# migmolper/NL-PartSol

Measured on AMD Instinct MI355X. Metric: particle-steps/sec (P2G+stress+G2P), higher is better.
Workload: dtype f64; 1 GPU; 3-D elastic cube impact, 1000000 particles/GPU (50x50x50 cells x 8 over 1 rank(s)), LME gamma=3, Neo-Hookean E=1e7 nu=0.3, explicit predictor-corrector step, 1xMI355X per rank; z-slabs for N>1 (weak scaling); particles_total=1000000, grid_nodes=226981, halo=none, halo_impl=none, library_default_resort_interval=50

## Files before the change

### nl-partsol_amd/csrc/nlps_gpu.hip

```cpp
#include <hip/hip_runtime.h>
#include <unistd.h>
#include <thread>
#include <hipcub/hipcub.hpp>

#include <dlfcn.h>
#include <rccl/rccl.h>

#include <algorithm>
#include <cmath>
#include <cstdio>
#include <cstdlib>
#include <cstring>
#include <numeric>
#include <map>
#include <string>
#include <type_traits>
#include <vector>

#include "../../include/nlps_gpu.h"
#include "nlps_device.hpp"
#include "nlps_tables.hpp"
#include "nlps_host_mem.hpp"

#define LAUNCH_ND_BLK(kern2, kern3, grid, block, ...)                                              \
// ... 226 lines not shown
      N.fixed[A * ND + a] = 0;
    }
  }
}

template <int ND>
__device__ __forceinline__ void dilate_node(int A, const GridD& g, const NView& N) {
  const int i0 = A % g.n[0], j0 = (A / g.n[0]) % g.n[1], k0 = A / (g.n[0] * g.n[1]);
  unsigned any = 0u;
#pragma unroll
  for (int dk = (ND == 3 ? -1 : 0); dk <= (ND == 3 ? 1 : 0); dk++)
#pragma unroll
    for (int dj = -1; dj <= 1; dj++)
#pragma unroll
      for (int di = -1; di <= 1; di++) {
        const int i = i0 + di, j = j0 + dj, k = k0 + dk;
        const bool ok = i >= 0 && i < g.n[0] && j >= 0 && j < g.n[1] && (ND == 2 || (k >= 0 && k < g.n[2]));
        if (ok) any |= N.seed[i + g.n[0] * (j + g.n[1] * k)];
      }
  N.active[A] = any ? 1 : 0;
}

template <int ND>
__device__ __forceinline__ int closest_node_update(const GridD& g, const uint8_t* __restrict__ rank1, const double* x, int I0) {
  int ijk[3] = {I0 % g.n[0], (I0 / g.n[0]) % g.n[1], I0 / (g.n[0] * g.n[1])};
  const uint8_t* rk = rank1 + 27 * class3_of<ND>(g, ijk);
  int sgn[3] = {0, 0, 0};
#pragma unroll
  for (int a = 0; a < ND; a++) {
    const double d = x[a] - (g.o[a] + g.h * (double)ijk[a]);
    if (fabs(d) > 0.49 * g.h) sgn[a] = d > 0.0 ? 1 : -1;
  }
  double best = 0.0;
  int bestrank = 256, bi = ijk[0], bj = ijk[1], bk = ijk[2];
#pragma unroll
  for (int q = 0; q < (1 << ND); q++) {
    const int di = (q & 1) ? sgn[0] : 0, dj = (q & 2) ? sgn[1] : 0, dk = (ND == 3 && (q & 4)) ? sgn[2] : 0;
    const bool dup = ((q & 1) && sgn[0] == 0) || ((q & 2) && sgn[1] == 0) || (ND == 3 && (q & 4) && sgn[2] == 0);
    const int i = ijk[0] + di, j = ijk[1] + dj, k = ijk[2] + dk;
    const bool ok = !dup && i >= 0 && i < g.n[0] && j >= 0 && j < g.n[1] && (ND == 2 || (k >= 0 && k < g.n[2]));
    if (ok) {
      double Dc = 0.0, t;
      t = x[0] - (g.o[0] + g.h * (double)i);
      Dc += t * t;
      t = x[1] - (g.o[1] + g.h * (double)j);
      Dc += t * t;
      if (ND == 3) {
        t = x[ND - 1] - (g.o[2] + g.h * (double)k);
        Dc += t * t;
      }
      const double d = sqrt(Dc);
      const int rank = rk[(di + 1) + 3 * (dj + 1) + 9 * (dk + 1)];
      if (bestrank == 256 || d < best || (d == best && rank < bestrank)) {
        best = d;
        bestrank = rank;
        bi = i;
        bj = j;
        bk = k;
      }
    }
  }
  return bi + g.n[0] * (bj + g.n[1] * bk);
}

template <int ND>
__global__ __launch_bounds__(BLK) void k_search(PView P, GridD g, NView N, const uint8_t* __restrict__ rank1, TileCnt tc,
                                                int update) {
  const int p = blockIdx.x * BLK + threadIdx.x;
  const bool valid = p < P.np;
  int I0 = 0;
  if (valid) {
    I0 = P.I0[p];
    if (update) {
      double x[ND], aux = 0.0;
#pragma unroll
      for (int a = 0; a < ND; a++) {
        x[a] = PF(P, F_X + a, p);
        aux += dsqr(PF(P, F_DIS + a, p));
      }
      if (sqrt(aux) > 0.0) {
        I0 = closest_node_update<ND>(g, rank1, x, I0);
        P.I0[p] = I0;
      }
      P.I0n[p] = I0;
    } else {
      const int In = P.I0n[p];
      if (In != I0) P.I0[p] = In;
      I0 = In;
    }
  }
  bin_particle<ND>(P, g, tc, p, I0, valid);
  if (valid && (!tc.count || P.tile[p] >= 0)) N.seed[I0] = 1;
}

template <int ND>
__global__ __launch_bounds__(BLK) void k_search_ahead(PView P, GridD g, NView N, const uint8_t* __restrict__ rank1, TileCnt tc) {
  const int p = blockIdx.x * BLK + threadIdx.x;
  int I0n = 0;
  bool binned = false;
  if (p < P.np) {
    I0n = P.I0[p];
    binned = P.tile[p] >= 0;
    if (binned && (P.mlo[p] | P.mhi[p]) != 0ull) {
      double xn[ND], dn2 = 0.0;
#pragma unroll
      for (int a = 0; a < ND; a++) {
        const double dd = PF(P, F_DDIS + a, p);
        xn[a] = PF(P, F_X + a, p) + dd;
        const double dn = PF(P, F_DIS + a, p) + dd;
        dn2 += dsqr(dn);
      }
      if (sqrt(dn2) > 0.0) I0n = closest_node_update<ND>(g, rank1, xn, I0n);
    }
    P.I0n[p] = I0n;
  }
  bin_particle<ND>(P, g, tc, binned ? p : P.np, I0n, binned);
  if (binned && P.tile[p] >= 0) N.seed[I0n] = 1;
}

__global__ void k_commit_I0(int np, const int* __restrict__ I0n, int* __restrict__ I0) {
  const int p = blockIdx.x * blockDim.x + threadIdx.x;
  if (p < np) I0[p] = I0n[p];
}

template <int ND>
__global__ __launch_bounds__(BLK) void k_init_I0(PView P, GridD g, NView N, TileCnt tc) {
  const int p = blockIdx.x * BLK + threadIdx.x;
  bool valid = p < P.np;
  int bestnode = 0;
  if (valid) {
    double x[ND];
    int c[3] = {0, 0, 0};
    bool found = true;
#pragma unroll
    for (int a = 0; a < ND; a++) {
      x[a] = PF(P, F_X + a, p);
      int nc = g.n[a] - 1;
      int ci = (int)floor((x[a] - g.o[a]) / g.h);
      ci = ci < 0 ? 0 : (ci > nc - 1 ? nc - 1 : ci);
      while (ci > 0 && x[a] <= g.o[a] + g.h * (double)ci) ci--;
// ... 1109 lines not shown
  bool rolled = false;
  bool level_b_fields = false;

  DevBuf<double> gridA;
  DevBuf<double> gridB;
  DevBuf<double> maskedA;

  std::vector<BcDev> bcs;
  DevBuf<unsigned> bcmask_d;

  DevBuf<int> perm_d;
  bool perm_dirty;
  int resort_every, steps_since_sort;
  DevBuf<unsigned long long> skey_d, skey2_d;
  DevBuf<int> sval_d, sval2_d;
  DevBuf<char> cub_tmp;
  size_t cub_tmp_bytes = 0;
  DevBuf<double> gather_tmp;
  DevBuf<double> Pd_alt;

  int nt[3], ntiles;
  DevBuf<int> tile_count_d;
  DevBuf<int> tile_count2_d;
  DevBuf<int> tile_start_d;
  DevBuf<int2> work1_d;
  DevBuf<int> node_cnt_d, nrank_d, tabo_d;
  DevBuf<int> tile_cursor_d;
  bool ranks_deferred = false;
  DevBuf<unsigned long long> tabm_d;
  DevBuf<int> home_d, foreign_d;
  Pinned<int> foreign_h;
  Pinned<int> status_h;
  bool rehome = true;
  double adaptive_resort = 0.8, debt = 0.0;
  int adaptive_min_steps = 4;
  DevBuf<int> nwork_d;
  DevBuf<int> dmg_first_d, dmg_last_d;
  DevBuf<int> dmg_first0_d, dmg_last0_d, dmg_sorted0_d;
  bool beps_snapshot = false;
  bool explicit_damage = false;
  int xl_n = 0, xl_nloads = 0;
  double xl_thickness = 1.0;
  DevBuf<int> xl_ids_d, xl_load_d, xl_inv_d;
  DevBuf<double> xl_a0_d, xl_T_d;
  bool xl_inv_valid = false, xl_lane_map = false;
  hipEvent_t xl_ev[2] = {};
// ... 399 lines not shown
  h->prm.tol_wrapper = prm->tol_wrapper_lme;
  h->prm.max_iter_lme = prm->max_iter_lme;
  h->prm.tol_radial = prm->tol_radial_returning;
  h->prm.max_iter_radial = prm->max_iter_radial_returning;
  h->P.erosion = prm->driver_eigenerosion != 0 || prm->driver_eigensoftening != 0;
  h->P.softening = prm->driver_eigensoftening != 0 && prm->driver_eigenerosion == 0;
#if NLPS_DEV
  if (const char* e = getenv("NLPS_LAZY_NODAL")) h->lazy_nodal = atoi(e);
#endif
  {
    int dev = 0, ncu = 0;
    if (hipGetDevice(&dev) == hipSuccess && hipDeviceGetAttribute(&ncu, hipDeviceAttributeMultiprocessorCount, dev) == hipSuccess && ncu > 0)
      h->ncu = ncu;
  }

  h->tab = nlps_host::build_tables(g.nd);
  HIPCHK(h->rank1_d.reserve(27 * 27));
  HIPCHK(hipMemcpy(h->rank1_d, h->tab.rank1, 27 * 27, hipMemcpyHostToDevice));

  size_t nn = (size_t)g.nnodes;
  int ND = g.nd;
  if (dev_alloc(h, h->N_active, nn, &h->N.active)) return 1;
  if (dev_alloc(h, h->N_seed, nn, &h->N.seed)) return 1;
  if (dev_alloc(h, h->N_nm, nn * (1 + ND), &h->N.nm)) return 1;
  if (dev_alloc(h, h->N_dU, nn * ND, &h->N.dU)) return 1;
  if (dev_alloc(h, h->N_force, nn * ND, &h->N.force)) return 1;
  if (dev_alloc(h, h->N_accel, nn * ND, &h->N.accel)) return 1;
  if (dev_alloc(h, h->N_reaction, nn * ND, &h->N.reaction)) return 1;
  if (dev_alloc(h, h->N_fixed, nn * ND, &h->N.fixed)) return 1;
  if (dev_alloc(h, h->h_avg_d, nn)) return 1;
  if (dev_alloc(h, h->n2m_d, nn)) return 1;
  if (dev_alloc(h, h->d2m_d, nn * ND)) return 1;
  if (dev_alloc(h, h->fixedm_d, nn * ND)) return 1;
  if (dev_alloc(h, h->bsum_d, nn * ND / 1024 + 2)) return 1;
  if (dev_alloc(h, h->total_d, 4)) return 1;
  if (dev_alloc(h, h->gstatus_d, 4)) return 1;
  if (dev_alloc(h, h->gridA, nn * 2 * ND)) return 1;
  if (dev_alloc(h, h->gridB, nn * 4 * ND)) return 1;
  {
    std::vector<double> hv;
    if (grid->h_avg) hv.assign(grid->h_avg, grid->h_avg + nn);
    else host_h_avg(*grid, h->tab, hv);
    HIPCHK(hipMemcpy(h->h_avg_d, hv.data(), nn * sizeof(double), hipMemcpyHostToDevice));
    h->N.h_avg = h->h_avg_d;
    HIPCHK(h->beta_t2_d.reserve(nn));
    hipLaunchKernelGGL(k_node_tables, dim3(nblk((int)nn)), dim3(BLK), 0, 0, (int)nn, (const double*)h->h_avg_d,
// ... 68 lines not shown
        used += m != 0;
        mixed += (m & (m - 1)) != 0;
      }
      h->k3_per_law = used > 0 && 4 * mixed <= used;
      if (h->law_present & ((1 << NLPS_KLAW_FRICTIONAL) | (1 << NLPS_KLAW_FLUID))) h->k3_per_law = 1;
    }
    std::stable_sort(h->perm.begin(), h->perm.end(), [&](int a, int b) { return key[a] < key[b]; });
    h->slab_lo = std::max(0, lo - 3);
    h->slab_hi = std::min(g.n[slab_axis] - 1, hi + 3);
  }
  if (dev_alloc(h, h->Pd, (size_t)NFD * h->P.npad, &h->P.d)) return 1;
  if (dev_alloc(h, h->P_I0, h->P.npad, &h->P.I0)) return 1;
  if (dev_alloc(h, h->P_I0n, h->P.npad, &h->P.I0n)) return 1;
  if (dev_alloc(h, h->P_mat, h->P.npad, &h->P.mat)) return 1;
  if (dev_alloc(h, h->P_nn, h->P.npad, &h->P.nn)) return 1;
  if (dev_alloc(h, h->P_status, h->P.npad, &h->P.status)) return 1;
  if (dev_alloc(h, h->P_mlo, h->P.npad, &h->P.mlo)) return 1;
  if (dev_alloc(h, h->P_mhi, h->P.npad, &h->P.mhi)) return 1;
  if (dev_alloc(h, h->P_tile, h->P.npad, &h->P.tile)) return 1;
  if (dev_alloc(h, h->P_rank, h->P.npad, &h->P.rank)) return 1;
  if (dev_alloc(h, h->order_d, h->P.npad)) return 1;
  if (dev_alloc(h, h->tile_count_d, (size_t)h->ntiles + 1)) return 1;
  if (dev_alloc(h, h->tile_count2_d, (size_t)h->ntiles + 1)) return 1;
  if (dev_alloc(h, h->tile_start_d, (size_t)h->ntiles + 1)) return 1;
  if (dev_alloc(h, h->work1_d, (size_t)h->ntiles)) return 1;
  if (dev_alloc(h, h->nwork_d, 6)) return 1;
#if NLPS_DEV
  if (const char* e = getenv("NLPS_ADAPTIVE_RESORT")) h->adaptive_resort = atof(e);
#endif
  if (dev_alloc(h, h->node_cnt_d, (size_t)h->g.nnodes)) return 1;
  if (dev_alloc(h, h->nrank_d, h->P.npad)) return 1;
  if (dev_alloc(h, h->tile_cursor_d, (size_t)h->ntiles + 1)) return 1;
  {
    const size_t nnw = h->g.nd == 3 ? TileTabCfg<3>::NNW : TileTabCfg<2>::NNW;
    if (dev_alloc(h, h->tabo_d, (size_t)h->ntiles * TileTab::LMAX * nnw)) return 1;
    if (dev_alloc(h, h->tabm_d, (size_t)h->ntiles * TileTab::LMAX * nnw)) return 1;
  }
  if (dev_alloc(h, h->home_d, h->P.npad)) return 1;
  if (dev_alloc(h, h->foreign_d, 64 * 32)) return 1;
  HIPCHK(h->foreign_h.alloc());
  *h->foreign_h.host() = 0;
  HIPCHK(h->status_h.alloc());
  *h->status_h.host() = 0;
#if NLPS_PHASE_TIMING
  if (dev_alloc(h, h->phase_d, 16 * 1024)) return 1;
#endif
  {
    std::vector<double> tmp(h->P.npad);
    int T = h->T;
    double idrow[9] = {0};
    idrow[0] = 1.0;
    idrow[ND + 1] = 1.0;
    idrow[T - 1] = 1.0;
// ... 1315 lines not shown
      td.slab_slot = -1;
      for_each_law_present(h->law_present, [&](int l, bool) {
        td.slab_slot++;
        launch_k3_law<MODE, true, 64>(h, td, l, a.dV);
      });
      return;
    }
  }
  if (per_law) {
    for_each_law_present(h->law_present, [&](int l, bool last) {
      if (a.signal && last) arm_signal(h, td, 1);
      launch_k3_law<MODE, true, K3_BLK>(h, td, l, a.dV);
    });
  } else if (law < 0) {
    if constexpr (K3Forms<MODE>::dispatch) {
      with_nd(h->nd, [&](auto D) { k3_go(h, k3_tile<CT(D), -1, MODE>, K3_BLK, td, no_rates); });
    }
  } else if (one_material_3d(h)) {
    with_law_in<1, 3>(law, [&](auto L) { k3_go(h, k3_tile<3, CT(L), MODE, false, K3_BLK, true>, K3_BLK, td, no_rates); });
  } else {
    launch_k3_law<MODE, false, K3_BLK>(h, td, law, a.dV);
  }
}
static void launch_k3_lazy(nlps_gpu* h, TileD td, bool signal, const LazyNodal& ln) {
  if (signal) arm_signal(h, td, 1);
  if (one_material_3d(h)) {
    with_law_in<1, 3>(h->uniform_law, [&](auto L) { k3_go(h, k3_tile_lazy<3, CT(L), true>, K3_BLK, td, ln); });
  } else {
    with_nd(h->nd, [&](auto D) {
      with_law(h->uniform_law, [&](auto L) { k3_go(h, k3_tile_lazy<CT(D), CT(L)>, K3_BLK, td, ln); });
    });
  }
}

template <int NF2, int NF3>
static void det_gather(nlps_gpu* h, int part, int slab_count, double* out) {
  const NodeRanges r = node_ranges(h, part);
  TileD tg = tile_view(h, 0);
  tg.slab_n = slab_count;
  if (r.an + r.bn > 0)
    LAUNCH_ND((k_slab_gather<2, NF2>), (k_slab_gather<3, NF3>), nblk(r.an + r.bn), r.a0, r.an, r.b0, r.bn, h->g, tg, out);
}
template <int NF2, int NF3, class F>
static int scatter_tiles(nlps_gpu* h, const char* who, int slab_count, double* out, F&& launch) {
  if (!det_implicit(h)) {
    launch(ic<BLK>{}, tile_view(h));
    return 0;
  }
  if (det_prepare(h, who)) return 1;
  launch(ic<64>{}, tile_view(h));
  det_gather<NF2, NF3>(h, 0, slab_count, out);
  return 0;
}
// ... 8 lines not shown
  }
  with_nd(h->nd, [&](auto D) {
    with_bool(p2g, [&](auto P2G) {
      hipLaunchKernelGGL((k2_tile<CT(D), CT(P2G)>), dim3(h->ntw), dim3(BLK), 0, h->stream, h->P, h->g, h->N, td,
                         h->prm, dt, gamma_nm, h->gstatus_d);
    });
  });
}

static int ensure_list_twins(nlps_gpu* h) {
  if (h->order_2_d) return 0;
  const size_t nn = (size_t)h->g.nnodes, ND = (size_t)h->nd;
  if (dev_alloc(h, h->work1_2_d, (size_t)h->ntiles)) return 1;
  if (dev_alloc(h, h->nwork2_d, 6)) return 1;
  if (dev_alloc(h, h->tile_start2_d, (size_t)h->ntiles + 1)) return 1;
  if (dev_alloc(h, h->order2_2_d, h->P.npad)) return 1;
  if (dev_alloc(h, h->N_active2, nn)) return 1;
  if (dev_alloc(h, h->N_fixed2, nn * ND)) return 1;
  if (dev_alloc(h, h->N_nm2, nn * (1 + ND))) return 1;
  if (dev_alloc(h, h->N_force2, nn * ND)) return 1;
  if (dev_alloc(h, h->order_2_d, h->P.npad)) return 1;
  return 0;
}
static void adopt_ready_lists(nlps_gpu* h) {
  h->work1_d.swap(h->work1_2_d);
  h->nwork_d.swap(h->nwork2_d);
  h->tile_start_d.swap(h->tile_start2_d);
  h->order_d.swap(h->order_2_d);
  h->order2_d.swap(h->order2_2_d);
  h->N_active.swap(h->N_active2);
  h->N_fixed.swap(h->N_fixed2);
  h->N_nm.swap(h->N_nm2);
  h->N_force.swap(h->N_force2);
  h->N.active = h->N_active;
  h->N.fixed = h->N_fixed;
  h->N.nm = h->N_nm;
  h->N.force = h->N_force;
  h->P_I0.swap(h->P_I0n);
  h->P.I0 = h->P_I0;
  h->P.I0n = h->P_I0n;
}

static int search_and_lists(nlps_gpu* h, bool init, bool p2g, double dt, double gamma_nm, int overlap = 0,
                            bool launch_lists_kernel = true) {
  int np = h->P.np;
  if (!p2g && materialise_nodal(h)) return 1;
  const bool ahead = h->ahead && !init, searched = h->searched;
  const bool deferred = ahead && h->ranks_deferred && node_lists(h);
  h->ranks_deferred = false;
  if (ahead) h->tile_count_d.swap(h->tile_count2_d);
  const bool ready = ahead && p2g && h->lists_ready;
  h->lists_ready = false;
  if (ready) adopt_ready_lists(h);
  if (ready) h->lists_exact = false;
  h->searched = h->ahead = false;
  if (!ready) {
  const bool clear_in_dilate = ahead && p2g;
  if (!clear_in_dilate)
    LAUNCH_ND((k_step_clear<2>), (k_step_clear<3>), nblk(std::max(h->nwn, h->ntw)), h->n0, h->nwn, h->N,
              h->tile_count_d + h->tile0, h->ntw, p2g ? 1 : 0, node_lists(h) ? h->node_cnt_d : nullptr, ahead ? 0 : 1);
  if (!ahead) {
    TileCnt tc = tile_cnt(h, true);
    if (init) LAUNCH_ND((k_init_I0<2>), (k_init_I0<3>), nblk(np), h->P, h->g, h->N, tc);
    else LAUNCH_ND((k_search<2>), (k_search<3>), nblk(np), h->P, h->g, h->N, h->rank1_d, tc, searched ? 0 : 1);
  }
  {
    const int TB = h->nd == 3 ? TileCfg<3>::TB : TileCfg<2>::TB;
    TileScanArgs ts{h->tile_count_d + h->tile0, h->tile_start_d + h->tile0, h->ntw, h->tile0, h->ntiles / h->nt[h->nd - 1], TB,
                    h->band_lo, h->band_hi, h->work1_d, h->nwork_d, deferred ? h->tile_cursor_d + h->tile0 : nullptr};
    const int nb = 1 + (h->nwn + 1023) / 1024 + (node_lists(h) ? (h->ntw + 15) / 16 : 0);
    int* fo = (h->adaptive_resort > 0.0 && !h->deterministic) ? h->foreign_d : nullptr;
    LAUNCH_ND_BLK(k_dilate_scan<2>, k_dilate_scan<3>, nb, 1024, h->n0, h->nwn, h->g, h->N, ts, fo, h->foreign_h.host(), tile_tab(h),
                  clear_in_dilate ? 1 : 0);
  }
  HIPCHK(hipGetLastError());
  if (halo(h, h->N.active, 1, 1, 1, overlap ? 1 : 0)) return 1;
// ... 980 lines not shown
    const NodeRanges in = node_ranges(h, 1);
    for (int i = 0; i < nbcc; i++) {
      if (h->bcs[i].n == 0) continue;
      double v[3];
      bc_values(bcc[i], step, h->nsteps, v);
      const int bits = dirbits_of(bcc[i], step, h->nsteps);
      const int r0 = part == 0 ? 0 : in.a0, r1 = part == 0 ? h->g.nnodes : in.a0 + in.an, inside = part == 2 ? 0 : 1;
      LAUNCH_ND(k_bc<2>, k_bc<3>, nblk(h->bcs[i].n), h->bcs[i].dnodes, h->bcs[i].n, bcc[i].dim, bits, v[0], v[1], v[2], h->N, r0,
                r1, inside);
    }
  }
  void nodal_accel(int part) {
    if (f.lazy) return;
    const NodeRanges r = node_ranges(h, part);
    int* ctile = (f.ride && !tiles_cleared) ? h->tile_count2_d + h->tile0 : nullptr;
    if (r.an + r.bn == 0 && !ctile) return;
    tiles_cleared = true;
    int* cnode = (f.ride && node_lists(h)) ? h->node_cnt_d.get() : nullptr;
    LAUNCH_ND(k_nodal_accel<2>, k_nodal_accel<3>, nblk(std::max(1, r.an + r.bn)), r.a0, r.an, r.b0, r.bn, h->N, gv[0], gv[1], gv[2],
              f.ride ? 1 : 0, cnode, ctile, h->ntw);
  }
  void k3(int cls, bool signal = false) {
    const TileD td = tile_view(h, cls);
    if (f.lazy) return launch_k3_lazy(h, td, signal, ln);
    const K3Launch a{signal, f.det && !f.dmg};
    if (f.dmg) launch_k3<5>(h, td, a);
    else launch_k3<1>(h, td, a);
  }
  void k5(int cls) {
    const TileD td = tile_view(h, cls);
    if (f.ride && !ks_made && !f.async_form) {
      ks.tc = tile_cnt(h, true);
      ks.tc.count = h->tile_count2_d;
      ks.tc.defer = node_lists(h) ? 1 : 0;
      h->ranks_deferred = ks.tc.defer != 0;
      ks_made = true;
    }
    const dim3 grid(h->ntw), blk(K5_BLK);
    with_nd(h->nd, [&](auto D) {
      with_bool(f.law == 0 || f.law == 1, [&](auto L01) {
        constexpr int LAW = CT(L01) ? 0 : 2;
        if (f.async_form) {
          hipLaunchKernelGGL((k5_tile_lazy<CT(D), LAW, false>), grid, blk, 0, h->stream, h->P, h->g, h->N, td, dt, gamma_nm, ks, ln,
                             h->gstatus_d);
        } else if (f.lazy) {
          hipLaunchKernelGGL((k5_tile_lazy<CT(D), LAW>), grid, blk, 0, h->stream, h->P, h->g, h->N, td, dt, gamma_nm, ks, ln,
                             h->gstatus_d);
        } else {
          with_bool(f.ride, [&](auto SEARCH) {
            hipLaunchKernelGGL((k5_tile<CT(D), LAW, CT(SEARCH)>), grid, blk, 0, h->stream, h->P, h->g, h->N, td, dt, gamma_nm, ks);
          });
        }
      });
    });
  }
  int search_next_and_fork() {
    const int np = h->P.np, ND = h->nd;
    TileCnt tc = tile_cnt(h, true);
    tc.count = h->tile_count2_d;
    h->ranks_deferred = false;
    LAUNCH_ND((k_search_ahead<2>), (k_search_ahead<3>), nblk(np), h->P, h->g, h->N, h->rank1_d, tc);
    HIPCHK(hipGetLastError());
    if (h->timing || resort_due(h)) return 0;
    if (ensure_list_twins(h)) return 1;
    HIPCHK(h->side.fork(h->stream));
    const hipStream_t ss = h->side.stream();
    const int TB = ND == 3 ? TileCfg<3>::TB : TileCfg<2>::TB;
    TileScanArgs ts{h->tile_count2_d + h->tile0, h->tile_start2_d + h->tile0, h->ntw, h->tile0, h->ntiles / h->nt[ND - 1], TB,
                    h->band_lo, h->band_hi, h->work1_2_d, h->nwork2_d, nullptr};
    NView N2 = h->N;
    N2.active = h->N_active2;
    N2.fixed = h->N_fixed2;
    N2.nm = h->N_nm2;
    N2.force = h->N_force2;
    constexpr int SNT = 256;
    const int nb = 1 + (h->nwn + SNT - 1) / SNT + (h->ntw + SNT / 64 - 1) / (SNT / 64);
    int* fo = h->adaptive_resort > 0.0 ? h->foreign_d : nullptr;
    with_nd(ND, [&](auto D) {
      hipLaunchKernelGGL((k_dilate_scan<CT(D), SNT>), dim3(nb), dim3(SNT), 0, ss, h->n0, h->nwn, h->g, N2, ts, fo, h->foreign_h.host(),
                         tile_tab(h), 1);
      hipLaunchKernelGGL(k_fill_orders<CT(D)>, dim3(nblk(np)), dim3(BLK), 0, ss, np, h->P.tile, h->P.rank, h->nrank_d, h->P.I0n,
                         (const int*)nullptr, h->tile_start2_d, h->g, tile_tab(h), h->order_2_d, h->order2_2_d, (int*)nullptr,
                         h->node_cnt_d);
    });
    HIPCHK(hipGetLastError());
    forked = true;
    return 0;
  }
  int damage_hook_and_forces() {
    if (damage_runs_and_hook(h, true)) return 1;
    if (f.det)
      LAUNCH_ND_BLK((k3f_wave<2, false>), (k3f_wave<3, false>), h->ntw, 64, h->P, h->g, h->N, tile_view(h, 0), h->gstatus_d);
    else
      LAUNCH_ND(k3f_tile<2>, k3f_tile<3>, h->ntw, h->P, h->g, h->N, tile_view(h, 0), h->gstatus_d);
    HIPCHK(hipGetLastError());
    return 0;
  }

  int run_overlap2() {
    const int ND = h->nd;
    if (halo(h, h->N.nm, 1 + ND, 8, 0, 3)) return 1;
    if (halo(h, h->N.nm, 1 + ND, 8, 0, 2)) return 1;
    nodal_dU(0);
    if (h->timing) HIPCHK(hipEventRecord(h->ev[3], h->stream));
    k3(0, true);
    HIPCHK(hipGetLastError());
// ... 18 lines not shown
    nodal_dU(2);
    k3(1);
    HIPCHK(hipGetLastError());
    if (h->timing) HIPCHK(hipEventRecord(h->ev[4], h->stream));
    gather_force(2);
    if (halo(h, h->N.force, ND, 8, 0, 1)) return 1;
    gather_force(1);
    nodal_accel(1);
    if (h->timing) HIPCHK(hipEventRecord(h->ev[5], h->stream));
    k5(2);
    if (halo(h, h->N.force, ND, 8, 0, 2)) return 1;
    nodal_accel(2);
    k5(1);
    HIPCHK(hipGetLastError());
    return 0;
  }
  int run_one_pass() {
    const int ND = h->nd, np = h->P.np;
    gather_nm(0);
    if (halo(h, h->N.nm, 1 + ND, 8, 0, 0)) return 1;
    nodal_dU(0);
    if (h->timing) HIPCHK(hipEventRecord(h->ev[3], h->stream));
    k3(0);
    if (f.dmg && np > 0 && damage_hook_and_forces()) return 1;
    HIPCHK(hipGetLastError());
    if (h->timing) HIPCHK(hipEventRecord(h->ev[4], h->stream));
    gather_force(0);
    if (f.loads && explicit_loads_launch(h, step)) return 1;
    if (halo(h, h->N.force, ND, 8, 0, 0)) return 1;
    nodal_accel(0);
    if (f.async_form && search_next_and_fork()) return 1;
    if (h->timing) HIPCHK(hipEventRecord(h->ev[5], h->stream));
    k5(0);
    if (f.dmg && np > 0) hipLaunchKernelGGL(k_damage_roll, dim3(nblk(np)), dim3(BLK), 0, h->stream, h->P);
    HIPCHK(hipGetLastError());
    if (forked) HIPCHK(h->side.join(h->stream));
    return 0;
  }
};

static int step_timing_read(nlps_gpu* h, bool loads) {
  HIPCHK(hipEventRecord(h->ev[6], h->stream));
  k3_go(h, k_null_bracket, BLK, tile_view(h, 0), no_rates);
  HIPCHK(hipEventRecord(h->ev[7], h->stream));
  HIPCHK(hipEventSynchronize(h->ev[7]));
  float t[7];
  for (int q = 0; q < 7; q++) HIPCHK(hipEventElapsedTime(&t[q], h->ev[q], h->ev[q + 1]));
  h->ms[0] = t[0];
  h->ms[1] = t[1];
  h->ms[2] = t[3];
  h->ms[3] = t[5];
  h->ms[4] = t[2] + t[4];
  h->ms[5] = t[6];
  h->ms[7] = 0.f;
// ... 1090 lines not shown
```

### nl-partsol_amd/csrc/nlps_tile_kernels.hpp

```cpp
#pragma once

#ifndef NLPS_DEV
#define NLPS_DEV 0
#endif
#if !NLPS_DEV && (defined(NLPS_ABL_ATOM) || defined(NLPS_ABL_GATHER) || defined(NLPS_PHASE_TIMING))
#error "NLPS_ABL_* / NLPS_PHASE_TIMING are developer experiments: build with -DNLPS_DEV=1 (tools/build_variant.sh)"
#endif

template <int ND>
struct TileCfg;
template <>
struct TileCfg<3> {
  static constexpr int TB = 4, W = 8, PS = 68, NW = 8 * 68;
  static constexpr int WA = 12, PSA = 100, NWA = 8 * 100;
};
template <>
struct TileCfg<2> {
  static constexpr int TB = 16, W = 20, PS = 400, NW = 400;
  static constexpr int WA = 20, PSA = 400, NWA = 400;
};

static constexpr int K3_BLK = 256, K5_BLK = 256;

struct TileD {
// ... 683 lines not shown
struct K3Waves {
  static constexpr int value = ND == 2 ? K3_WAVES_2D
                               : ((MODE == 1 || MODE == 3 || MODE == 5 || MODE == 6) && LAW == NLPS_MAT_NEO_HOOKEAN) ? K3_WAVES_NH
                               : ((MODE == 1 || MODE == 3 || MODE == 5 || MODE == 6) && LAW == NLPS_MAT_HENCKY)      ? K3_WAVES_HENCKY
                               : ((MODE == 1 || MODE == 3 || MODE == 5 || MODE == 6) && LAW == NLPS_MAT_DRUCKER_PRAGER) ? K3_WAVES_DP
                                                                               : K3_WAVES;
};
template <int ND, int MODE, bool FILT>
struct K3Lds {
  static constexpr int NW = TileCfg<ND>::NW, NWA = TileCfg<ND>::NWA;
  static constexpr bool RATES = (MODE == 2 || MODE == 4);
  static constexpr int SELCAP = FILT ? 4096 : 1;
  static constexpr int N_DVXY = RATES ? 2 * NW : 2, N_DVZ = (RATES && ND == 3) ? NW : 1, N_DUZ = (ND == 3) ? NW : 1;
  static constexpr int N_FAC = (MODE == 6) ? 1 : ND * NWA;
  double* dvxy;
  double* dvz;
  double* duxy;
  double* duz;
  double* fac;
  int* sel;
  int* nsel;
  int* wcnt;
};
template <int ND, int LAW, int MODE, bool FILT, int NT, bool UMAT = false>
__device__ __forceinline__ void k3_body(const PView& P, const GridD& g, const NView& N, const TileD& td,
                                        const MatD* __restrict__ mats, const ParamsD& prm, int* __restrict__ gstatus,
                                        const double* __restrict__ dVgrid, const TileWork& tw, int nbnd,
                                        const K3Lds<ND, MODE, FILT>& lds, const NodalFold* fs) {
  NLPS_FP_CONTRACT
  constexpr int W = TileCfg<ND>::W, PS = TileCfg<ND>::PS, NW = TileCfg<ND>::NW, KN = Lme<ND>::KN;
  constexpr bool RATES = (MODE == 2 || MODE == 4);
  constexpr bool SCATTER = (MODE == 1 || MODE == 3 || MODE == 4);
  constexpr bool STATE = (MODE == 5);
  constexpr bool STATE_N1 = (MODE == 6);
  constexpr bool STRESS = SCATTER || STATE || STATE_N1;
  static_assert((MODE == 4) == (LAW == NLPS_KLAW_FLUID), "the rate-carrying residual is the fluid law's, and only its");
  double* const dvxy = lds.dvxy;
  double* const dvz = lds.dvz;
  double* const duxy = lds.duxy;
  double* const duz = lds.duz;
  double* const fac = lds.fac;
  int* const sel = lds.sel;
  int& nsel = *lds.nsel;
  int* const wcnt = lds.wcnt;
  constexpr int WA = TileCfg<ND>::WA, PSA = TileCfg<ND>::PSA, NWA = TileCfg<ND>::NWA;
  const int wb = tw.wb, tile = tw.tile;
  int cnt = td.count[tile];
  PH_INIT
  constexpr int SELCAP = FILT ? 4096 : 1;
  bool listed = false;
  if (FILT) {
    const int start0 = td.start[tile];
// ... 59 lines not shown
    } else {
      duxy[2 * idx] = in ? N.dU[(size_t)node * ND + 0] : 0.0;
      duxy[2 * idx + 1] = in ? N.dU[(size_t)node * ND + 1] : 0.0;
      if (ND == 3) duz[(ND == 3) ? idx : 0] = in ? N.dU[(size_t)node * ND + (2 % ND)] : 0.0;
    }
    if (RATES) {
      dvxy[RATES ? 2 * idx : 0] = in ? dVgrid[(size_t)node * ND + 0] : 0.0;
      dvxy[RATES ? 2 * idx + 1 : 1] = in ? dVgrid[(size_t)node * ND + 1] : 0.0;
      if (ND == 3) dvz[(RATES && ND == 3) ? idx : 0] = in ? dVgrid[(size_t)node * ND + (2 % ND)] : 0.0;
    }
  }
  if (!STATE_N1)
    for (int idx = threadIdx.x; idx < ND * NWA; idx += NT) fac[idx] = 0.0;
  __syncthreads();
  const double2* du2 = reinterpret_cast<const double2*>(duxy);
  const double2* dv2 = reinterpret_cast<const double2*>(dvxy);
  const int start = td.start[tile];
  PH(8)
  for (int s = threadIdx.x; s < cnt; s += NT) {
    const int p = (FILT && listed) ? sel[FILT ? s : 0] : td.order[start + s];
    if (FILT && !listed && mats[P.mat[p]].type != LAW) continue;
    Lme<ND> c;
    double lam[ND], beta;
    if (!load_lme<ND>(P, g, p, c, lam, beta)) continue;
    const int mat_idx = UMAT ? 0 : (STRESS ? P.mat[p] : -1);
    const int base = window_base<ND>(c.ijk, w0);
    NLPS_YZ_LOCALS(c);
    PH(9)
    double Z = 0.0, rx = 0.0, ry = 0.0, rz = 0.0, Jxx = 0.0, Jxy = 0.0, Jxz = 0.0, Jyy = 0.0, Jyz = 0.0, Jzz = 0.0;
    double G[ND * ND], Gv[RATES ? ND * ND : 1];
    double U[ND];
    double Uv[RATES ? ND : 1];
#pragma unroll
    for (int a = 0; a < ND; a++) U[a] = 0.0;
#pragma unroll
    for (int a = 0; a < (RATES ? ND : 1); a++) Uv[a] = 0.0;
#pragma unroll
    for (int a = 0; a < ND * ND; a++) G[a] = 0.0;
#pragma unroll
    for (int a = 0; a < (RATES ? ND * ND : 1); a++) Gv[a] = 0.0;
    constexpr bool TWOPASS = ND == 3 && STRESS && K3Waves<ND, LAW, MODE>::value >= 3;
    double Fn[ND * ND], fzz = 0.0;
    if (TWOPASS) {
#pragma unroll 1
      for (int k = 0; k < KN; k++) {
        const unsigned pb = plane_bits<ND>(c, k);
        const int basek = base + PS * (k - 2);
// ... 281 lines not shown
      for (int i = 0; i < ND; i++)
#pragma unroll
        for (int j = 0; j < ND; j++) {
          double a2 = 0.0;
#pragma unroll
          for (int k2 = 0; k2 < ND; k2++) a2 += dDF[i * ND + k2] * Fn[k2 * ND + j] + DF[i * ND + k2] * dFn[k2 * ND + j];
          dFn1[i * ND + j] = a2;
        }
      store_block<ND>(P, F_DTDF, pl, dDF, 0.0, false);
      store_block<ND>(P, F_DTFN1, pl, dFn1, 0.0, false);
      if (MODE == 4) {
#pragma unroll
        for (int q = 0; q < ND * ND; q++) dFk[q % ((MODE == 4) ? ND * ND : 1)] = dFn1[q];
      }
    }
    if (!STRESS) {
      if (st) {
        atomicOr(&P.status[pl], st);
        atomicOr(gstatus, st);
      }
      continue;
    }
    if (MODE == 1 || STATE) {
#pragma unroll
      for (int a = 0; a < ND; a++) PF(P, F_DDIS + a, pl) = U[a] * Zinv;
    }
    if constexpr (STATE) {
      if (PF(P, F_DMG, pl) == 1.0) {
        PF(P, F_W, pl) = 0.0;
        const int lw = (LAW >= 0) ? LAW : mats[mat_idx].type;
        if (lw != NLPS_MAT_NEO_HOOKEAN && lw != NLPS_MAT_HENCKY) {
#pragma unroll
          for (int q = 0; q < ((ND == 2) ? 5 : 9); q++) PF(P, fBEN1(P) + q, pl) = PF(P, fBEN(P) + q, pl);
        }
      } else {
        double tau_s[ND * ND];
        st |= stress_update<ND, LAW, false, (LAW == NLPS_KLAW_FRICTIONAL), true, true>(P, pl, mats, prm, Fn1, DF, Jn1, tau_s, mat_idx);
      }
      if (st) {
        atomicOr(&P.status[pl], st);
        atomicOr(gstatus, st);
      }
      continue;
    }
    if constexpr (STATE_N1) {
      if (PF(P, F_DMG, pl) == 1.0) {
        PF(P, F_W, pl) = 0.0;
      } else {
// ... 118 lines not shown
  __shared__ __attribute__((aligned(16))) double dvxy[L::N_DVXY];
  __shared__ double dvz[L::N_DVZ];
  __shared__ __attribute__((aligned(16))) double duxy[2 * L::NW];
  __shared__ double duz[L::N_DUZ];
  __shared__ double fac[L::N_FAC];
  __shared__ int sel[L::SELCAP];
  __shared__ int nsel;
  __shared__ int wcnt[NT / 64];
  const int nbnd = (MODE == 1 || MODE >= 3) ? tile_boundary_count(td) : 0;
  if (MODE == 1 || MODE >= 3) tile_signal_empty(td, nbnd);
  TileWork tw;
  if (!tile_work_item(td, tw)) return;
  const L lds{dvxy, dvz, duxy, duz, fac, sel, &nsel, wcnt};
  k3_body<ND, LAW, MODE, FILT, NT, UMAT>(P, g, N, td, mats, prm, gstatus, dVgrid, tw, nbnd, lds, nullptr);
}

struct LazyNodal {
  NodalFold fs;
  int n0, nwn;
  int* node_cnt;
  int* tile_count;
  int ntw;
};
template <int ND, int LAW, bool UMAT = false>
__global__ __launch_bounds__(K3_BLK, (K3Waves<ND, LAW, 1>::value)) void k3_tile_lazy(PView P, GridD g, NView N, TileD td, const MatD* __restrict__ mats,
                                                                                  ParamsD prm, int* __restrict__ gstatus, LazyNodal ln) {
  using L = K3Lds<ND, 1, false>;
  __shared__ __attribute__((aligned(16))) double dvxy[L::N_DVXY];
  __shared__ double dvz[L::N_DVZ];
  __shared__ __attribute__((aligned(16))) double duxy[2 * L::NW];
  __shared__ double duz[L::N_DUZ];
  __shared__ double fac[ND * L::NWA];
  __shared__ int sel[L::SELCAP];
  __shared__ int nsel;
  __shared__ int wcnt[K3_BLK / 64];
  for (int i = blockIdx.x * K3_BLK + threadIdx.x; i < max(ln.nwn, ln.ntw); i += gridDim.x * K3_BLK) {
    if (i < ln.ntw) ln.tile_count[i] = 0;
    if (i < ln.nwn) {
      N.seed[ln.n0 + i] = 0;
      if (ln.node_cnt) ln.node_cnt[ln.n0 + i] = 0;
    }
  }
  const int nbnd = tile_boundary_count(td);
  tile_signal_empty(td, nbnd);
  TileWork tw;
  if (!tile_work_item(td, tw)) return;
  const L lds{dvxy, dvz, duxy, duz, fac, sel, &nsel, wcnt};
  k3_body<ND, LAW, 1, false, K3_BLK, UMAT>(P, g, N, td, mats, prm, gstatus, nullptr, tw, nbnd, lds, &ln.fs);
}

template <int ND, bool PLUS = false>
__global__ __launch_bounds__(K3_BLK, 2) void k3f_tile(PView P, GridD g, NView N, TileD td, int* __restrict__ gstatus) {
  NLPS_FP_CONTRACT
  constexpr int KN = Lme<ND>::KN, WA = TileCfg<ND>::WA, PSA = TileCfg<ND>::PSA, NWA = TileCfg<ND>::NWA;
  __shared__ double fac[ND * NWA];
  TileWork tw;
  if (!tile_work_item(td, tw)) return;
  const int tile = tw.tile, cnt = td.count[tile];
  int w0[3];
  tile_origin<ND>(td, tile, w0);
  for (int idx = threadIdx.x; idx < ND * NWA; idx += K3_BLK) fac[idx] = 0.0;
  __syncthreads();
  const int start = td.start[tile];
  for (int s = threadIdx.x; s < cnt; s += K3_BLK) {
    const int p = td.order[start + s];
    Lme<ND> c;
    double lam[ND], beta;
    if (!load_lme<ND>(P, g, p, c, lam, beta)) continue;
    double Zinv, r[ND], J[ND * ND], Jm1[ND * ND], tau[ND * ND], DF[ND * ND], B[ND * ND], z;
    lme_moments_h<ND>(c, Zinv, r, J);
    load_block<ND>(P, F_TAU, p, tau, z);
// ... 587 lines not shown
```

Measured before the change: 1.635 billion particle-steps/s.

## Fold next-step neighbor search and binning into the lazy k3 stress kernel

Removes the separate k_search_ahead kernel and performs the closest-node walk, tile binning, node counting and seeding for the next step inside the k3 lazy kernel, right after each particle's displacement increment is computed. Counts go into double-buffered tile/node/seed arrays that are swapped after launch, and the side-stream list fork now starts right after k3 instead of after nodal acceleration, so it overlaps with the later stages. This avoids a full pass over particle positions and a kernel launch, but adds atomics and register pressure to the already heavy stress kernel.

After: 1.614 billion particle-steps/s. 1.3% lower.

```diff
diff --git a/nl-partsol_amd/csrc/nlps_gpu.hip b/nl-partsol_amd/csrc/nlps_gpu.hip
--- a/nl-partsol_amd/csrc/nlps_gpu.hip
+++ b/nl-partsol_amd/csrc/nlps_gpu.hip
@@ -272,8 +272,8 @@
 }
 
 template <int ND>
-__device__ __forceinline__ int closest_node_update(const GridD& g, const uint8_t* __restrict__ rank1, const double* x, int I0) {
-  int ijk[3] = {I0 % g.n[0], (I0 / g.n[0]) % g.n[1], I0 / (g.n[0] * g.n[1])};
+__device__ __forceinline__ int closest_node_walk(const GridD& g, const uint8_t* __restrict__ rank1, const double* x, const int* ijk,
+                                                 int* win) {
   const uint8_t* rk = rank1 + 27 * class3_of<ND>(g, ijk);
   int sgn[3] = {0, 0, 0};
 #pragma unroll
@@ -310,7 +310,16 @@
       }
     }
   }
+  win[0] = bi;
+  win[1] = bj;
+  win[2] = bk;
   return bi + g.n[0] * (bj + g.n[1] * bk);
+}
+template <int ND>
+__device__ __forceinline__ int closest_node_update(const GridD& g, const uint8_t* __restrict__ rank1, const double* x, int I0) {
+  const int ijk[3] = {I0 % g.n[0], (I0 / g.n[0]) % g.n[1], I0 / (g.n[0] * g.n[1])};
+  int win[3];
+  return closest_node_walk<ND>(g, rank1, x, ijk, win);
 }
 
 template <int ND>
@@ -341,31 +350,6 @@
   }
   bin_particle<ND>(P, g, tc, p, I0, valid);
   if (valid && (!tc.count || P.tile[p] >= 0)) N.seed[I0] = 1;
-}
-
-template <int ND>
-__global__ __launch_bounds__(BLK) void k_search_ahead(PView P, GridD g, NView N, const uint8_t* __restrict__ rank1, TileCnt tc) {
-  const int p = blockIdx.x * BLK + threadIdx.x;
-  int I0n = 0;
-  bool binned = false;
-  if (p < P.np) {
-    I0n = P.I0[p];
-    binned = P.tile[p] >= 0;
-    if (binned && (P.mlo[p] | P.mhi[p]) != 0ull) {
-      double xn[ND], dn2 = 0.0;
-#pragma unroll
-      for (int a = 0; a < ND; a++) {
-        const double dd = PF(P, F_DDIS + a, p);
-        xn[a] = PF(P, F_X + a, p) + dd;
-        const double dn = PF(P, F_DIS + a, p) + dd;
-        dn2 += dsqr(dn);
-      }
-      if (sqrt(dn2) > 0.0) I0n = closest_node_update<ND>(g, rank1, xn, I0n);
-    }
-    P.I0n[p] = I0n;
-  }
-  bin_particle<ND>(P, g, tc, binned ? p : P.np, I0n, binned);
-  if (binned && P.tile[p] >= 0) N.seed[I0n] = 1;
 }
 
 __global__ void k_commit_I0(int np, const int* __restrict__ I0n, int* __restrict__ I0) {
@@ -1521,6 +1505,8 @@
   int nt[3], ntiles;
   DevBuf<int> tile_count_d;
   DevBuf<int> tile_count2_d;
+  DevBuf<int> tile_count3_d, node_cnt2_d;
+  DevBuf<unsigned char> N_seed2;
   DevBuf<int> tile_start_d;
   DevBuf<int2> work1_d;
   DevBuf<int> node_cnt_d, nrank_d, tabo_d;
@@ -1966,6 +1952,7 @@
   int ND = g.nd;
   if (dev_alloc(h, h->N_active, nn, &h->N.active)) return 1;
   if (dev_alloc(h, h->N_seed, nn, &h->N.seed)) return 1;
+  if (dev_alloc(h, h->N_seed2, nn)) return 1;
   if (dev_alloc(h, h->N_nm, nn * (1 + ND), &h->N.nm)) return 1;
   if (dev_alloc(h, h->N_dU, nn * ND, &h->N.dU)) return 1;
   if (dev_alloc(h, h->N_force, nn * ND, &h->N.force)) return 1;
@@ -2080,6 +2067,7 @@
   if (dev_alloc(h, h->order_d, h->P.npad)) return 1;
   if (dev_alloc(h, h->tile_count_d, (size_t)h->ntiles + 1)) return 1;
   if (dev_alloc(h, h->tile_count2_d, (size_t)h->ntiles + 1)) return 1;
+  if (dev_alloc(h, h->tile_count3_d, (size_t)h->ntiles + 1)) return 1;
   if (dev_alloc(h, h->tile_start_d, (size_t)h->ntiles + 1)) return 1;
   if (dev_alloc(h, h->work1_d, (size_t)h->ntiles)) return 1;
   if (dev_alloc(h, h->nwork_d, 6)) return 1;
@@ -2087,6 +2075,7 @@
   if (const char* e = getenv("NLPS_ADAPTIVE_RESORT")) h->adaptive_resort = atof(e);
 #endif
   if (dev_alloc(h, h->node_cnt_d, (size_t)h->g.nnodes)) return 1;
+  if (dev_alloc(h, h->node_cnt2_d, (size_t)h->g.nnodes)) return 1;
   if (dev_alloc(h, h->nrank_d, h->P.npad)) return 1;
   if (dev_alloc(h, h->tile_cursor_d, (size_t)h->ntiles + 1)) return 1;
   {
@@ -3448,13 +3437,15 @@
     launch_k3_law<MODE, false, K3_BLK>(h, td, law, a.dV);
   }
 }
-static void launch_k3_lazy(nlps_gpu* h, TileD td, bool signal, const LazyNodal& ln) {
+template <class LN>
+static void launch_k3_lazy(nlps_gpu* h, TileD td, bool signal, const LN& ln) {
+  constexpr bool SEARCH = std::is_same<LN, LazySearch>::value;
   if (signal) arm_signal(h, td, 1);
   if (one_material_3d(h)) {
-    with_law_in<1, 3>(h->uniform_law, [&](auto L) { k3_go(h, k3_tile_lazy<3, CT(L), true>, K3_BLK, td, ln); });
+    with_law_in<1, 3>(h->uniform_law, [&](auto L) { k3_go(h, k3_tile_lazy<3, CT(L), true, SEARCH>, K3_BLK, td, ln); });
   } else {
     with_nd(h->nd, [&](auto D) {
-      with_law(h->uniform_law, [&](auto L) { k3_go(h, k3_tile_lazy<CT(D), CT(L)>, K3_BLK, td, ln); });
+      with_law(h->uniform_law, [&](auto L) { k3_go(h, k3_tile_lazy<CT(D), CT(L), false, SEARCH>, K3_BLK, td, ln); });
     });
   }
 }
@@ -3509,20 +3500,22 @@
   if (dev_alloc(h, h->order_2_d, h->P.npad)) return 1;
   return 0;
 }
-static void adopt_ready_lists(nlps_gpu* h) {
+static void adopt_ready_lists(nlps_gpu* h, bool nodal) {
   h->work1_d.swap(h->work1_2_d);
   h->nwork_d.swap(h->nwork2_d);
   h->tile_start_d.swap(h->tile_start2_d);
   h->order_d.swap(h->order_2_d);
   h->order2_d.swap(h->order2_2_d);
   h->N_active.swap(h->N_active2);
-  h->N_fixed.swap(h->N_fixed2);
-  h->N_nm.swap(h->N_nm2);
-  h->N_force.swap(h->N_force2);
   h->N.active = h->N_active;
-  h->N.fixed = h->N_fixed;
-  h->N.nm = h->N_nm;
-  h->N.force = h->N_force;
+  if (nodal) {
+    h->N_fixed.swap(h->N_fixed2);
+    h->N_nm.swap(h->N_nm2);
+    h->N_force.swap(h->N_force2);
+    h->N.fixed = h->N_fixed;
+    h->N.nm = h->N_nm;
+    h->N.force = h->N_force;
+  }
   h->P_I0.swap(h->P_I0n);
   h->P.I0 = h->P_I0;
   h->P.I0n = h->P_I0n;
@@ -3536,9 +3529,9 @@
   const bool deferred = ahead && h->ranks_deferred && node_lists(h);
   h->ranks_deferred = false;
   if (ahead) h->tile_count_d.swap(h->tile_count2_d);
-  const bool ready = ahead && p2g && h->lists_ready;
+  const bool ready = ahead && h->lists_ready;
   h->lists_ready = false;
-  if (ready) adopt_ready_lists(h);
+  if (ready) adopt_ready_lists(h, p2g);
   if (ready) h->lists_exact = false;
   h->searched = h->ahead = false;
   if (!ready) {
@@ -4565,6 +4558,23 @@
   }
   void k3(int cls, bool signal = false) {
     const TileD td = tile_view(h, cls);
+    if (f.async_form) {
+      LazySearch ls;
+      static_cast<LazyNodal&>(ls) = ln;
+      ls.ks.rank1 = h->rank1_d;
+      ls.ks.tc = tile_cnt(h, true);
+      ls.ks.tc.count = h->tile_count3_d;
+      ls.ks.tc.node_cnt = h->node_cnt2_d;
+      ls.ks.tc.defer = 1;
+      ls.ks.seed = h->N_seed2;
+      h->ranks_deferred = true;
+      launch_k3_lazy(h, td, signal, ls);
+      h->tile_count2_d.swap(h->tile_count3_d);
+      h->node_cnt_d.swap(h->node_cnt2_d);
+      h->N_seed.swap(h->N_seed2);
+      h->N.seed = h->N_seed;
+      return;
+    }
     if (f.lazy) return launch_k3_lazy(h, td, signal, ln);
     const K3Launch a{signal, f.det && !f.dmg};
     if (f.dmg) launch_k3<5>(h, td, a);
@@ -4597,20 +4607,15 @@
       });
     });
   }
-  int search_next_and_fork() {
+  int fork_lists() {
     const int np = h->P.np, ND = h->nd;
-    TileCnt tc = tile_cnt(h, true);
-    tc.count = h->tile_count2_d;
-    h->ranks_deferred = false;
-    LAUNCH_ND((k_search_ahead<2>), (k_search_ahead<3>), nblk(np), h->P, h->g, h->N, h->rank1_d, tc);
-    HIPCHK(hipGetLastError());
     if (h->timing || resort_due(h)) return 0;
     if (ensure_list_twins(h)) return 1;
     HIPCHK(h->side.fork(h->stream));
     const hipStream_t ss = h->side.stream();
     const int TB = ND == 3 ? TileCfg<3>::TB : TileCfg<2>::TB;
     TileScanArgs ts{h->tile_count2_d + h->tile0, h->tile_start2_d + h->tile0, h->ntw, h->tile0, h->ntiles / h->nt[ND - 1], TB,
-                    h->band_lo, h->band_hi, h->work1_2_d, h->nwork2_d, nullptr};
+                    h->band_lo, h->band_hi, h->work1_2_d, h->nwork2_d, h->tile_cursor_d + h->tile0};
     NView N2 = h->N;
     N2.active = h->N_active2;
     N2.fixed = h->N_fixed2;
@@ -4623,8 +4628,8 @@
       hipLaunchKernelGGL((k_dilate_scan<CT(D), SNT>), dim3(nb), dim3(SNT), 0, ss, h->n0, h->nwn, h->g, N2, ts, fo, h->foreign_h.host(),
                          tile_tab(h), 1);
       hipLaunchKernelGGL(k_fill_orders<CT(D)>, dim3(nblk(np)), dim3(BLK), 0, ss, np, h->P.tile, h->P.rank, h->nrank_d, h->P.I0n,
-                         (const int*)nullptr, h->tile_start2_d, h->g, tile_tab(h), h->order_2_d, h->order2_2_d, (int*)nullptr,
-                         h->node_cnt_d);
+                         (const int*)nullptr, h->tile_start2_d, h->g, tile_tab(h), h->order_2_d, h->order2_2_d,
+                         h->tile_cursor_d.get(), h->node_cnt_d);
     });
     HIPCHK(hipGetLastError());
     forked = true;
@@ -4689,6 +4694,7 @@
     nodal_dU(0);
     if (h->timing) HIPCHK(hipEventRecord(h->ev[3], h->stream));
     k3(0);
+    if (f.async_form && fork_lists()) return 1;
     if (f.dmg && np > 0 && damage_hook_and_forces()) return 1;
     HIPCHK(hipGetLastError());
     if (h->timing) HIPCHK(hipEventRecord(h->ev[4], h->stream));
@@ -4696,7 +4702,6 @@
     if (f.loads && explicit_loads_launch(h, step)) return 1;
     if (halo(h, h->N.force, ND, 8, 0, 0)) return 1;
     nodal_accel(0);
-    if (f.async_form && search_next_and_fork()) return 1;
     if (h->timing) HIPCHK(hipEventRecord(h->ev[5], h->stream));
     k5(0);
     if (f.dmg && np > 0) hipLaunchKernelGGL(k_damage_roll, dim3(nblk(np)), dim3(BLK), 0, h->stream, h->P);
diff --git a/nl-partsol_amd/csrc/nlps_tile_kernels.hpp b/nl-partsol_amd/csrc/nlps_tile_kernels.hpp
--- a/nl-partsol_amd/csrc/nlps_tile_kernels.hpp
+++ b/nl-partsol_amd/csrc/nlps_tile_kernels.hpp
@@ -729,12 +729,61 @@
   int* nsel;
   int* wcnt;
 };
-template <int ND, int LAW, int MODE, bool FILT, int NT, bool UMAT = false>
+struct K3Search {
+  const uint8_t* rank1;
+  TileCnt tc;
+  unsigned char* seed;
+};
+template <int ND>
+__device__ __forceinline__ void k3_count_next(const PView& P, const K3Search& ks, int p, int I0n, const int* win, int tile) {
+  constexpr int TB = TileCfg<ND>::TB;
+  const TileCnt& tc = ks.tc;
+  const int t = (win[0] / TB) + tc.nt[0] * ((win[1] / TB) + tc.nt[1] * (ND == 3 ? win[2] / TB : 0));
+  const int lane = threadIdx.x & 63;
+  const bool stay = t == tile;
+  const u64 ms = __ballot(stay);
+  if (stay) {
+    if (lane == __ffsll((unsigned long long)ms) - 1) atomicAdd(&tc.count[tile], (int)__popcll(ms));
+  } else {
+    atomicAdd(&tc.count[t], 1);
+  }
+  P.I0n[p] = I0n;
+  P.tile[p] = t;
+  atomicAdd(&tc.node_cnt[I0n], 1);
+  ks.seed[I0n] = 1;
+  if (tc.home) {
+    bool away = false;
+    if (tc.rehome) tc.home[p] = t;
+    else away = t != tc.home[p];
+    const u64 m = __ballot(away);
+    if (away && lane == __ffsll((unsigned long long)m) - 1)
+      atomicAdd(&tc.foreign[32 * ((blockIdx.x * (blockDim.x >> 6) + (threadIdx.x >> 6)) & 63)], (int)__popcll(m));
+  }
+}
+template <int ND>
+__device__ __forceinline__ void k3_search_next(const PView& P, const GridD& g, const K3Search& ks, int p, const double* dd,
+                                               int I0, const int* ijk, int tile) {
+#pragma clang fp contract(off)
+  double xn[ND], dn2 = 0.0;
+#pragma unroll
+  for (int a = 0; a < ND; a++) {
+    xn[a] = PF(P, F_X + a, p) + dd[a];
+    const double dn = PF(P, F_DIS + a, p) + dd[a];
+    dn2 += dsqr(dn);
+  }
+  int I0n = I0, win[3] = {ijk[0], ijk[1], ijk[2]};
+  if (sqrt(dn2) > 0.0) I0n = closest_node_walk<ND>(g, ks.rank1, xn, ijk, win);
+  k3_count_next<ND>(P, ks, p, I0n, win, tile);
+}
+
+template <int ND, int LAW, int MODE, bool FILT, int NT, bool UMAT = false, bool SEARCH = false>
 __device__ __forceinline__ void k3_body(const PView& P, const GridD& g, const NView& N, const TileD& td,
                                         const MatD* __restrict__ mats, const ParamsD& prm, int* __restrict__ gstatus,
                                         const double* __restrict__ dVgrid, const TileWork& tw, int nbnd,
-                                        const K3Lds<ND, MODE, FILT>& lds, const NodalFold* fs) {
+                                        const K3Lds<ND, MODE, FILT>& lds, const NodalFold* fs,
+                                        const K3Search* ksr = nullptr) {
   NLPS_FP_CONTRACT
+  static_assert(!SEARCH || (MODE == 1 && !FILT), "the search of the next step belongs to the folded explicit step (K3Search)");
   constexpr int W = TileCfg<ND>::W, PS = TileCfg<ND>::PS, NW = TileCfg<ND>::NW, KN = Lme<ND>::KN;
   constexpr bool RATES = (MODE == 2 || MODE == 4);
   constexpr bool SCATTER = (MODE == 1 || MODE == 3 || MODE == 4);
@@ -840,7 +889,10 @@
     if (FILT && !listed && mats[P.mat[p]].type != LAW) continue;
     Lme<ND> c;
     double lam[ND], beta;
-    if (!load_lme<ND>(P, g, p, c, lam, beta)) continue;
+    if (!load_lme<ND>(P, g, p, c, lam, beta)) {
+      if constexpr (SEARCH) k3_count_next<ND>(P, *ksr, p, c.I0, c.ijk, tile);
+      continue;
+    }
     const int mat_idx = UMAT ? 0 : (STRESS ? P.mat[p] : -1);
     const int base = window_base<ND>(c.ijk, w0);
     NLPS_YZ_LOCALS(c);
@@ -1168,8 +1220,10 @@
       continue;
     }
     if (MODE == 1 || STATE) {
-#pragma unroll
-      for (int a = 0; a < ND; a++) PF(P, F_DDIS + a, pl) = U[a] * Zinv;
+      double dd[ND];
+#pragma unroll
+      for (int a = 0; a < ND; a++) PF(P, F_DDIS + a, pl) = dd[a] = U[a] * Zinv;
+      if constexpr (SEARCH) k3_search_next<ND>(P, g, *ksr, pl, dd, c.I0, c.ijk, tile);
     }
     if constexpr (STATE) {
       if (PF(P, F_DMG, pl) == 1.0) {
@@ -1334,9 +1388,13 @@
   int* tile_count;
   int ntw;
 };
-template <int ND, int LAW, bool UMAT = false>
+struct LazySearch : LazyNodal {
+  K3Search ks;
+};
+template <int ND, int LAW, bool UMAT = false, bool SEARCH = false>
 __global__ __launch_bounds__(K3_BLK, (K3Waves<ND, LAW, 1>::value)) void k3_tile_lazy(PView P, GridD g, NView N, TileD td, const MatD* __restrict__ mats,
-                                                                                  ParamsD prm, int* __restrict__ gstatus, LazyNodal ln) {
+                                                                                  ParamsD prm, int* __restrict__ gstatus,
+                                                                                  std::conditional_t<SEARCH, LazySearch, LazyNodal> ln) {
   using L = K3Lds<ND, 1, false>;
   __shared__ __attribute__((aligned(16))) double dvxy[L::N_DVXY];
   __shared__ double dvz[L::N_DVZ];
@@ -1358,7 +1416,9 @@
   TileWork tw;
   if (!tile_work_item(td, tw)) return;
   const L lds{dvxy, dvz, duxy, duz, fac, sel, &nsel, wcnt};
-  k3_body<ND, LAW, 1, false, K3_BLK, UMAT>(P, g, N, td, mats, prm, gstatus, nullptr, tw, nbnd, lds, &ln.fs);
+  const K3Search* ksr = nullptr;
+  if constexpr (SEARCH) ksr = &ln.ks;
+  k3_body<ND, LAW, 1, false, K3_BLK, UMAT, SEARCH>(P, g, N, td, mats, prm, gstatus, nullptr, tw, nbnd, lds, &ln.fs, ksr);
 }
 
 template <int ND, bool PLUS = false>
```
